# alibaba/VideoMV

Hardware: AMD Instinct MI355X
Metric: denoise-steps/sec, t2v 320x512x24 (latent 24x40x64), CFG 9.0, 50-step DDIM schedule (higher is better)
Workload: dtype fp16; 1 GPU; t2v_infer.yaml UNetSD_T2VBase 1.413B, 24 views, latent 40x64, 77 ctx tokens, 1 sample per GPU (cond+uncond batched); parallelism=replicas x1

## Files before the change

### include/vmv.h

```cpp
#ifndef VMV_H
#define VMV_H
#include <stdint.h>
#include <stddef.h>

#ifdef __cplusplus
extern "C" {
#endif

#define VMV_OK            0
#define VMV_EINVAL       -1
#define VMV_EALIGN       -2
#define VMV_ENULL        -3
#define VMV_ERANGE       -4
#define VMV_ECOMM        -5

#define VMV_ABI_VERSION   12
int vmv_abi_version(void);
#define VMV_ELEM_F16      0
#define VMV_ELEM_BF16     1
int vmv_elem_type(void);
int vmv_has_experiments(void);
int vmv_sizeof(int which);
const char* vmv_error_string(int code);

// ... 67 lines not shown
#define VMV_TILE_PP256x160 12
#define VMV_TILE_Q128x128 13
#define VMV_TILE_Q96x160  14
#define VMV_TILE_S256x128 15
#define VMV_TILE_S192x160 16
#define VMV_TILE_S256x160 17
#define VMV_TILE_A128x160 18
#define VMV_TILE_A128x128 19
#define VMV_TILE_X256x320 20
#define VMV_TILE_X256x256 21
#define VMV_TILE_X256x128 22
#define VMV_TILE_RS       23
#define VMV_TILE_RS512    24
#define VMV_TILE_RS256    25
#define VMV_TILE_HALO     26
#define VMV_TILE_TFR      27

#define VMV_TILE_TQA      28
#define VMV_TILE_W256x256 29

#define VMV_TILE_X512x128 30
#define VMV_TILE_Y256x128 31

#define VMV_TILE_TRS      32

int vmv_gemm(const VmvGemmParams* p, void* stream);
int vmv_gemm_tqa_ok(const VmvGemmParams* p);
int vmv_gemm_up4_ok(const VmvGemmParams* p);
int vmv_gemm_ln_inline_ok(const VmvGemmParams* p);
int vmv_gemm_rs_ok(const VmvGemmParams* p);
int vmv_gemm_tfr_ok(const VmvGemmParams* p);
int vmv_gemm_trs_ok(const VmvGemmParams* p);
int vmv_gemm_trs_blocks(const VmvGemmParams* p, int max_blocks, void* stream);
int vmv_gemm_pick_tile(const VmvGemmParams* p);
int vmv_gemm_validate(const VmvGemmParams* p);
int vmv_gemm_served_tile(const VmvGemmParams* p);
int vmv_gemm_tile_map(int bid, int tiles_m, int tiles_n, int gm, int* tile_m, int* tile_n);
int vmv_gemm_group_m(int tiles_m, int tiles_n, int BM, int BN, int conc);

typedef struct {
    int32_t M, C;
    const void* x; int32_t ldx;
    int32_t _pad0;
    const void* w1;
    const float* b1;
    const void* w2;
    const float* b2;
    const void* residual; int32_t ldr;
    float ln_eps;
    void* out; int32_t ldo;
    int32_t _pad1;
} VmvFfParams;
int vmv_ff_fused(const VmvFfParams* p, void* stream);
int vmv_ff_fused_ok(const VmvFfParams* p);

typedef struct {
    const void* x;
    const void* x1;
    int32_t ld, ld1;
    int32_t C0, C1;
    int32_t rows, rows_per_stat;
    int32_t chunk_rows;
    float* partial;
    const float* gamma;
    const float* beta;
    float eps;
    int32_t silu;
    void* y;
    int32_t ldy;
    int32_t fold_ranks;
    int64_t* totals;
    int64_t* totals_clear;
    int32_t clear_count;
    int32_t _pad;
} VmvGroupNormParams;

#define VMV_GN_REC 8
#define VMV_GN_NREP 8
int vmv_groupnorm_stats(const VmvGroupNormParams* p, void* stream);
int vmv_groupnorm_table(const VmvGroupNormParams* p, void* stream);
int vmv_groupnorm_apply(const VmvGroupNormParams* p, void* stream);
#define VMV_GN_FUSED_BYTES 131072
int vmv_groupnorm_fused(const VmvGroupNormParams* p, int32_t cols, void* stream);

typedef struct {
    const void* x; int32_t ldx;
    void* y; int32_t ldy;
    const float* gamma; const float* beta;
    int32_t rows, C;
    float eps;
    int32_t _pad;
    float* stats_out;
} VmvLayerNormParams;
int vmv_layernorm(const VmvLayerNormParams* p, void* stream);

typedef struct {
    const float* s; int32_t lds;
    void* p; int32_t ldp;
    int32_t rows, n;
    float scale;
    int32_t _pad;
} VmvSoftmaxParams;
int vmv_softmax_rows(const VmvSoftmaxParams* p, void* stream);

typedef struct {
    int64_t s_outer, s_inner, s_row;
    int32_t inner; int32_t _pad;
} VmvSeqMap;

typedef struct {
    const void* q; const void* k; const void* v; void* o;
    VmvSeqMap qm, km, vm, om;
    int32_t n_outer;
    int32_t kv_div;
    int32_t heads;
    int32_t Nq, Nk;
    float scale;
    int32_t head_dim;
    int32_t causal;
} VmvAttnParams;
int vmv_attention(const VmvAttnParams* p, void* stream);
#define VMV_ATTN_SHORT    1
#define VMV_ATTN_WAVE     2
#define VMV_ATTN_Q128     3
#define VMV_ATTN_Q256     4
#define VMV_ATTN_CAUSAL   5
#define VMV_ATTN_D32      6
#define VMV_ATTN_D128     7
int vmv_attention_served_kernel(const VmvAttnParams* p);

int vmv_latent_to_rows(const float* x, void* rows, int nb_src, int C, int F, int H, int W, int Cpad, int nrep,
                       void* stream);
int vmv_latent_to_rows_keep(const float* x, void* rows, int nb, int C, int F, int H, int W, int ld, int nrep, void* stream);
int vmv_rows_to_nchw(const void* rows, int rows_fp32, int ld, float* out, int n, int C, int HW, void* stream);

typedef struct {
    const float* eps_rows;
    int32_t ld;
    int32_t C, F, HW;
    float guide_scale;
    float c_recip, c_recipm1;
    float c_sqrt_ac, c_sqrt_1mac;
    float a_prev;
    int32_t v_pred;
    float* xt;
    float* x0_out;
    float clamp;
    float sigma;
    const float* noise;
} VmvDdimParams;
int vmv_cfg_ddim_step(const VmvDdimParams* p, void* stream);

int vmv_posterior_sample(const float* moments_rows, int ld, const float* noise, float* z, int n, int zc, int HW, float scale,
                         void* stream);
int vmv_emb_combine_silu(const float* temb, const float* cam, void* out, int rows, int C, int rows_per_t,
                         int cam_rows, void* stream);
int vmv_sinusoidal(const float* t, void* out_elem, int n, int dim, void* stream);

int vmv_i2v_temporal_adapter(const void* in, int ld_in, void* out, int ld_out, const float* w, int F, int HW, int nrep,
                             float scale, void* stream);
int vmv_adaptive_avgpool_rows(const void* in, int ld, void* out, int ldo, int n, int C, int IH, int IW, int OH, int OW,
                              void* stream);

int vmv_lgm_x0_views(const float* eps_rows, int ld, int branch, const float* xt, int C, int F, int HW, const int32_t* idx4,
                     float c_recip, float c_recipm1, float inv_scale, float* out, void* stream);
int vmv_lgm_pack_input(const float* decoded, const float* rays, float* out, int nviews, int HW, void* stream);
// ... 211 lines not shown
```

### videomv_amd/_lib.py

```python
import ctypes as C
import os

_HERE = os.path.dirname(os.path.abspath(__file__))
_ELEM_NAMES = {"fp16": "f16", "f16": "f16", "float16": "f16", "half": "f16", "bf16": "bf16", "bfloat16": "bf16"}
_elem = _ELEM_NAMES[os.environ.get("VMV_DTYPE", "fp16").lower()]
ELEM_F16, ELEM_BF16 = 0, 1


def set_elem(name: str):
    global _elem
    new = _ELEM_NAMES[str(name).lower()]
    if _lib is not None and new != _elem:
        raise RuntimeError(f"the {_elem} kernels are already loaded; set VMV_DTYPE / call set_elem() before first use")
    _elem = new


def elem_name() -> str:
    return "fp16" if _elem == "f16" else "bf16"


def elem():
    import torch
    return torch.float16 if _elem == "f16" else torch.bfloat16


def lib_path() -> str:
    return os.path.join(os.environ.get("VMV_LIB_DIR") or os.path.join(_HERE, "lib"), f"libvmv_hip_{_elem}.so")

VMV_MAX_SEGS = 24
SEG_LINEAR, SEG_SPATIAL, SEG_TEMPORAL = 0, 1, 2
EPI_NONE, EPI_GEGLU, EPI_TATTN = 0, 1, 2
ACT_NONE, ACT_SILU, ACT_GELU = 0, 1, 2
TILE_AUTO, TILE_128x128, TILE_128x160, TILE_128x64, TILE_64x64, TILE_256x128, TILE_256x160 = 0, 1, 2, 3, 4, 5, 6
TILE_G128x128, TILE_G128x160, TILE_P256x128, TILE_P256x160, TILE_PP256x128, TILE_PP256x160 = 7, 8, 9, 10, 11, 12
TILE_Q128x128, TILE_Q96x160 = 13, 14
TILE_S256x128, TILE_S192x160, TILE_S256x160 = 15, 16, 17
TILE_A128x160, TILE_A128x128 = 18, 19
TILE_X256x320, TILE_X256x256, TILE_X256x128 = 20, 21, 22
TILE_RS, TILE_RS512, TILE_RS256, TILE_HALO, TILE_TFR, TILE_TQA, TILE_W256x256, TILE_X512x128, TILE_Y256x128 = 23, 24, 25, 26, 27, 28, 29, 30, 31
TRS_TILE = 32
OP_GEMM, OP_GN_STATS, OP_GN_APPLY, OP_LAYERNORM, OP_ATTENTION, OP_SOFTMAX, OP_COPY, OP_GN_FUSED, OP_FF, OP_GN_TABLE, OP_COMM = 1, 2, 3, 4, 5, 6, 7, 8, 9, 10, 11
COMM_ALL_TO_ALL, COMM_ALL_GATHER, COMM_ID_BYTES = 0, 1, 128
ABI_VERSION = 12
ATTN_SHORT, ATTN_WAVE, ATTN_Q128, ATTN_Q256, ATTN_CAUSAL, ATTN_D32, ATTN_D128 = 1, 2, 3, 4, 5, 6, 7
GN_FUSED_BYTES = 131072


class GemmSeg(C.Structure):
    _fields_ = [("src", C.c_void_p), ("ld", C.c_int32), ("k", C.c_int32), ("mode", C.c_int32),
                ("d0", C.c_int32), ("d1", C.c_int32), ("_pad", C.c_int32)]


class GemmParams(C.Structure):
    _fields_ = [("M", C.c_int32), ("N", C.c_int32), ("nseg", C.c_int32), ("ktot", C.c_int32),
                ("seg", GemmSeg * VMV_MAX_SEGS),
                ("W", C.c_void_p), ("bias", C.c_void_p), ("rowvec", C.c_void_p),
                ("rowvec_div", C.c_int32), ("rowvec_ld", C.c_int32),
                ("residual", C.c_void_p), ("ldr", C.c_int32),
                ("epilogue", C.c_int32), ("act", C.c_int32), ("out_fp32", C.c_int32),
                ("out", C.c_void_p), ("ldo", C.c_int32),
                ("OH", C.c_int32), ("OW", C.c_int32), ("IH", C.c_int32), ("IW", C.c_int32),
                ("stride", C.c_int32), ("ups", C.c_int32),
                ("F", C.c_int32), ("P", C.c_int32),
                ("ksplit", C.c_int32), ("workspace", C.c_void_p),
                ("tile", C.c_int32), ("res_scale", C.c_float), ("rowstat", C.c_void_p), ("colsum", C.c_void_p),
                ("ln_eps", C.c_float), ("wgroup_rows", C.c_int32), ("wgroup_stride", C.c_int64),
                ("gn_table", C.c_void_p), ("gn_rows_per_stat", C.c_int32), ("gn_silu", C.c_int32), ("epi_scale", C.c_float),
                ("phased", C.c_int32)]


class GroupNormParams(C.Structure):
    _fields_ = [("x", C.c_void_p), ("x1", C.c_void_p), ("ld", C.c_int32), ("ld1", C.c_int32),
                ("C0", C.c_int32), ("C1", C.c_int32), ("rows", C.c_int32), ("rows_per_stat", C.c_int32),
                ("chunk_rows", C.c_int32), ("partial", C.c_void_p), ("gamma", C.c_void_p), ("beta", C.c_void_p),
                ("eps", C.c_float), ("silu", C.c_int32), ("y", C.c_void_p), ("ldy", C.c_int32), ("fold_ranks", C.c_int32),
                ("totals", C.c_void_p), ("totals_clear", C.c_void_p), ("clear_count", C.c_int32), ("_pad", C.c_int32)]


class FfParams(C.Structure):
    _fields_ = [("M", C.c_int32), ("C", C.c_int32), ("x", C.c_void_p), ("ldx", C.c_int32), ("_pad0", C.c_int32),
                ("w1", C.c_void_p), ("b1", C.c_void_p), ("w2", C.c_void_p), ("b2", C.c_void_p),
                ("residual", C.c_void_p), ("ldr", C.c_int32), ("ln_eps", C.c_float),
                ("out", C.c_void_p), ("ldo", C.c_int32), ("_pad1", C.c_int32)]


class GsParams(C.Structure):
    _fields_ = [("gaussians", C.c_void_p), ("N", C.c_int32), ("size", C.c_int32), ("view", C.c_void_p),
                ("view_proj", C.c_void_p), ("tan_half_fov", C.c_float), ("bg", C.c_float * 3),
                ("depth", C.c_void_p), ("xy", C.c_void_p), ("conic_opacity", C.c_void_p), ("rect", C.c_void_p),
                ("tiles_touched", C.c_void_p), ("offsets", C.c_void_p), ("scan_temp", C.c_void_p),
                ("scan_temp_bytes", C.c_size_t), ("keys", C.c_void_p), ("keys_sorted", C.c_void_p), ("vals", C.c_void_p),
                ("vals_sorted", C.c_void_p), ("num_rendered", C.c_int32), ("_pad", C.c_int32), ("sort_temp", C.c_void_p),
                ("sort_temp_bytes", C.c_size_t), ("ranges", C.c_void_p), ("out_color", C.c_void_p), ("out_alpha", C.c_void_p)]


class GsBatchParams(C.Structure):
    _fields_ = [("gaussians", C.c_void_p), ("B", C.c_int32), ("N", C.c_int32), ("V", C.c_int32), ("size", C.c_int32),
                ("views", C.c_void_p), ("view_projs", C.c_void_p), ("tan_half_fov", C.c_float), ("bg", C.c_float * 3),
                ("depth", C.c_void_p), ("xy", C.c_void_p), ("conic_opacity", C.c_void_p), ("rect", C.c_void_p),
                ("tiles_touched", C.c_void_p), ("offsets", C.c_void_p), ("scan_temp", C.c_void_p),
                ("scan_temp_bytes", C.c_size_t), ("keys", C.c_void_p), ("keys_sorted", C.c_void_p), ("vals", C.c_void_p),
                ("vals_sorted", C.c_void_p), ("num_rendered", C.c_int32), ("_pad", C.c_int32), ("sort_temp", C.c_void_p),
                ("sort_temp_bytes", C.c_size_t), ("ranges", C.c_void_p), ("out_color", C.c_void_p), ("out_alpha", C.c_void_p)]


class GsBackwardParams(C.Structure):
    _fields_ = [("pass_", GsBatchParams), ("final_T", C.c_void_p), ("n_contrib", C.c_void_p), ("dL_dimage", C.c_void_p),
                ("grad2d", C.c_void_p), ("grad_view", C.c_void_p), ("grad", C.c_void_p)]


class GsDepthParams(C.Structure):
    _fields_ = [("pass_", GsBatchParams), ("out_depth", C.c_void_p), ("out_median_depth", C.c_void_p)]


class GsAdamParams(C.Structure):
    _fields_ = [("params", C.c_void_p), ("m", C.c_void_p), ("v", C.c_void_p), ("grad", C.c_void_p), ("gaussians", C.c_void_p),
                ("n", C.c_int32), ("step", C.c_int32), ("lr", C.c_float * 5), ("beta1", C.c_float), ("beta2", C.c_float),
                ("eps", C.c_float)]


class GsSsimLossParams(C.Structure):
    _fields_ = [("image", C.c_void_p), ("target", C.c_void_p), ("planes", C.c_int32), ("height", C.c_int32), ("width", C.c_int32),
                ("lambda_dssim", C.c_float), ("dL_dimage", C.c_void_p), ("loss", C.c_void_p), ("workspace", C.c_void_p),
                ("workspace_bytes", C.c_size_t)]


class GsTsdfParams(C.Structure):
    _fields_ = [("depth", C.c_void_p), ("colour", C.c_void_p), ("views", C.c_void_p), ("n_views", C.c_int), ("size", C.c_int),
# ... 4 lines not shown
class GsMeshComponentsParams(C.Structure):
    _fields_ = [("faces", C.c_void_p), ("face_stride", C.c_int64), ("n_faces", C.c_int64), ("n_vertices", C.c_int64),
                ("label", C.c_void_p), ("face_count", C.c_void_p), ("status", C.c_void_p)]


class GsMeshBakeParams(C.Structure):
    _fields_ = [("verts", C.c_void_p), ("vert_colours", C.c_void_p), ("faces", C.c_void_p), ("face_stride", C.c_int64),
                ("n_faces", C.c_int64), ("n_vertices", C.c_int64), ("depth", C.c_void_p), ("colour", C.c_void_p), ("views", C.c_void_p),
                ("n_views", C.c_int32), ("size", C.c_int32), ("tan_half_fov", C.c_float), ("z_min", C.c_float), ("depth_tol", C.c_float),
                ("cos_min", C.c_float), ("patch", C.c_int32), ("tex_size", C.c_int32), ("out", C.c_void_p), ("plane_stride", C.c_int64),
                ("status", C.c_void_p)]


MESH_STATUS_RANGE, MESH_STATUS_GAVE_UP = 1, 2


class CopyParams(C.Structure):
    _fields_ = [("src", C.c_void_p), ("dst", C.c_void_p), ("n0", C.c_int32), ("n1", C.c_int32), ("n2", C.c_int32),
                ("inner16", C.c_int32), ("ss0", C.c_int64), ("ss1", C.c_int64), ("ss2", C.c_int64)]


class CommParams(C.Structure):
    _fields_ = [("comm", C.c_void_p), ("kind", C.c_int32), ("_pad", C.c_int32), ("send", C.c_void_p), ("recv", C.c_void_p),
                ("bytes", C.c_int64)]


class LayerNormParams(C.Structure):
    _fields_ = [("x", C.c_void_p), ("ldx", C.c_int32), ("y", C.c_void_p), ("ldy", C.c_int32),
                ("gamma", C.c_void_p), ("beta", C.c_void_p), ("rows", C.c_int32), ("C", C.c_int32),
                ("eps", C.c_float), ("_pad", C.c_int32), ("stats_out", C.c_void_p)]


class SeqMap(C.Structure):
    _fields_ = [("s_outer", C.c_int64), ("s_inner", C.c_int64), ("s_row", C.c_int64),
                ("inner", C.c_int32), ("_pad", C.c_int32)]


class AttnParams(C.Structure):
    _fields_ = [("q", C.c_void_p), ("k", C.c_void_p), ("v", C.c_void_p), ("o", C.c_void_p),
                ("qm", SeqMap), ("km", SeqMap), ("vm", SeqMap), ("om", SeqMap),
                ("n_outer", C.c_int32), ("kv_div", C.c_int32), ("heads", C.c_int32),
                ("Nq", C.c_int32), ("Nk", C.c_int32), ("scale", C.c_float), ("head_dim", C.c_int32), ("causal", C.c_int32)]


class SoftmaxParams(C.Structure):
    _fields_ = [("s", C.c_void_p), ("lds", C.c_int32), ("p", C.c_void_p), ("ldp", C.c_int32),
                ("rows", C.c_int32), ("n", C.c_int32), ("scale", C.c_float), ("_pad", C.c_int32)]


class DdimParams(C.Structure):
    _fields_ = [("eps_rows", C.c_void_p), ("ld", C.c_int32), ("C", C.c_int32), ("F", C.c_int32), ("HW", C.c_int32),
                ("guide_scale", C.c_float), ("c_recip", C.c_float), ("c_recipm1", C.c_float),
                ("c_sqrt_ac", C.c_float), ("c_sqrt_1mac", C.c_float), ("a_prev", C.c_float),
                ("v_pred", C.c_int32), ("xt", C.c_void_p), ("x0_out", C.c_void_p),
                ("clamp", C.c_float), ("sigma", C.c_float), ("noise", C.c_void_p)]


_P = C.c_void_p
SYMBOLS = {
    "vmv_abi_version": (C.c_int, []),
    "vmv_elem_type": (C.c_int, []),
    "vmv_sizeof": (C.c_int, [C.c_int]),
    "vmv_error_string": (C.c_char_p, [C.c_int]),
    "vmv_gemm": (C.c_int, [C.POINTER(GemmParams), _P]),
    "vmv_gemm_ln_inline_ok": (C.c_int, [C.POINTER(GemmParams)]),
    "vmv_gemm_rs_ok": (C.c_int, [C.POINTER(GemmParams)]),
    "vmv_gemm_tfr_ok": (C.c_int, [C.POINTER(GemmParams)]),
    "vmv_gemm_tqa_ok": (C.c_int, [C.POINTER(GemmParams)]),
    "vmv_gemm_trs_ok": (C.c_int, [C.POINTER(GemmParams)]),
    "vmv_gemm_trs_blocks": (C.c_int, [C.POINTER(GemmParams), C.c_int, _P]),
    "vmv_gemm_up4_ok": (C.c_int, [C.POINTER(GemmParams)]),
    "vmv_has_experiments": (C.c_int, []),
    "vmv_ff_fused": (C.c_int, [C.POINTER(FfParams), _P]),
    "vmv_ff_fused_ok": (C.c_int, [C.POINTER(FfParams)]),
    "vmv_gemm_pick_tile": (C.c_int, [C.POINTER(GemmParams)]),
    "vmv_gemm_validate": (C.c_int, [C.POINTER(GemmParams)]),
    "vmv_gemm_served_tile": (C.c_int, [C.POINTER(GemmParams)]),
    "vmv_gemm_tile_map": (C.c_int, [C.c_int, C.c_int, C.c_int, C.c_int, C.POINTER(C.c_int), C.POINTER(C.c_int)]),
    "vmv_gemm_group_m": (C.c_int, [C.c_int, C.c_int, C.c_int, C.c_int, C.c_int]),
    "vmv_groupnorm_stats": (C.c_int, [C.POINTER(GroupNormParams), _P]),
    "vmv_groupnorm_apply": (C.c_int, [C.POINTER(GroupNormParams), _P]),
    "vmv_groupnorm_table": (C.c_int, [C.POINTER(GroupNormParams), _P]),
    "vmv_groupnorm_fused": (C.c_int, [C.POINTER(GroupNormParams), C.c_int32, _P]),
    "vmv_layernorm": (C.c_int, [C.POINTER(LayerNormParams), _P]),
    "vmv_attention": (C.c_int, [C.POINTER(AttnParams), _P]),
    "vmv_attention_served_kernel": (C.c_int, [C.POINTER(AttnParams)]),
    "vmv_softmax_rows": (C.c_int, [C.POINTER(SoftmaxParams), _P]),
    "vmv_permute_copy": (C.c_int, [C.POINTER(CopyParams), _P]),
    "vmv_gaussian_activation": (C.c_int, [_P, C.c_int, _P, C.c_int, _P, _P]),
    "vmv_lgm_x0_views": (C.c_int, [_P, C.c_int, C.c_int, _P, C.c_int, C.c_int, C.c_int, _P, C.c_float, C.c_float, C.c_float, _P, _P]),
    "vmv_lgm_pack_input": (C.c_int, [_P, _P, _P, C.c_int, C.c_int, _P]),
    "vmv_lgm_render_to_vae": (C.c_int, [_P, _P, C.c_int, C.c_int, C.c_int, _P]),
    "vmv_ddim_x0_step": (C.c_int, [_P, _P, _P, C.c_long, C.c_float, C.c_float, C.c_float, C.c_float, C.c_float, C.c_float, _P, _P]),
    "vmv_gs_workspace_bytes": (C.c_int, [C.c_int, C.c_int, C.POINTER(C.c_size_t), C.POINTER(C.c_size_t)]),
    "vmv_gs_preprocess": (C.c_int, [C.POINTER(GsParams), _P]),
    "vmv_gs_render": (C.c_int, [C.POINTER(GsParams), _P]),
    "vmv_gs_batch_key_bits": (C.c_int, [C.c_int, C.c_int]),
    "vmv_gs_batch_workspace_bytes": (C.c_int, [C.c_int, C.c_int, C.c_int, C.POINTER(C.c_size_t), C.POINTER(C.c_size_t)]),
    "vmv_gs_batch_preprocess": (C.c_int, [C.POINTER(GsBatchParams), _P]),
    "vmv_gs_batch_render": (C.c_int, [C.POINTER(GsBatchParams), _P]),
    "vmv_gs_batch_render_depth": (C.c_int, [C.POINTER(GsDepthParams), _P]),
    "vmv_gs_batch_render_state": (C.c_int, [C.POINTER(GsBackwardParams), _P]),
    "vmv_gs_batch_backward": (C.c_int, [C.POINTER(GsBackwardParams), _P]),
    "vmv_gs_image_loss": (C.c_int, [_P, _P, C.c_long, _P, _P, _P, _P]),
    "vmv_gs_adam_step": (C.c_int, [C.POINTER(GsAdamParams), _P]),
    "vmv_gs_ssim_loss_workspace_bytes": (C.c_int, [C.c_int, C.c_int, C.c_int, C.POINTER(C.c_size_t)]),
    "vmv_gs_ssim_loss": (C.c_int, [C.POINTER(GsSsimLossParams), _P]),
    "vmv_gs_tsdf_integrate": (C.c_int, [C.POINTER(GsTsdfParams), _P]),
    "vmv_gs_mesh_components": (C.c_int, [C.POINTER(GsMeshComponentsParams), _P]),
    "vmv_gs_mesh_bake": (C.c_int, [C.POINTER(GsMeshBakeParams), _P]),
    "vmv_latent_to_rows": (C.c_int, [_P, _P, C.c_int, C.c_int, C.c_int, C.c_int, C.c_int, C.c_int, C.c_int, _P]),
    "vmv_latent_to_rows_keep": (C.c_int, [_P, _P, C.c_int, C.c_int, C.c_int, C.c_int, C.c_int, C.c_int, C.c_int, _P]),
    "vmv_i2v_temporal_adapter": (C.c_int, [_P, C.c_int, _P, C.c_int, _P, C.c_int, C.c_int, C.c_int, C.c_float, _P]),
    "vmv_adaptive_avgpool_rows": (C.c_int, [_P, C.c_int, _P, C.c_int, C.c_int, C.c_int, C.c_int, C.c_int, C.c_int, C.c_int, _P]),
    "vmv_rows_to_nchw": (C.c_int, [_P, C.c_int, C.c_int, _P, C.c_int, C.c_int, C.c_int, _P]),
    "vmv_cfg_ddim_step": (C.c_int, [C.POINTER(DdimParams), _P]),
    "vmv_posterior_sample": (C.c_int, [_P, C.c_int, _P, _P, C.c_int, C.c_int, C.c_int, C.c_float, _P]),
    "vmv_emb_combine_silu": (C.c_int, [_P, _P, _P, C.c_int, C.c_int, C.c_int, C.c_int, _P]),
    "vmv_sinusoidal": (C.c_int, [_P, _P, C.c_int, C.c_int, _P]),
    "vmv_plan_create": (_P, []),
    "vmv_plan_destroy": (None, [_P]),
    "vmv_plan_add": (C.c_int, [_P, C.c_int, _P, C.c_size_t]),
    "vmv_plan_size": (C.c_int, [_P]),
    "vmv_plan_run": (C.c_int, [_P, _P]),
    "vmv_plan_run_range": (C.c_int, [_P, C.c_int, C.c_int, _P]),
    "vmv_plan_capture": (_P, [_P, _P]),
    "vmv_graph_launch": (C.c_int, [_P, _P]),
    "vmv_graph_nodes": (C.c_int, [_P]),
    "vmv_graph_destroy": (None, [_P]),
    "vmv_comm_load": (C.c_int, [C.c_char_p]),
    "vmv_comm_loaded": (C.c_int, []),
    "vmv_comm_unique_id": (C.c_int, [_P]),
    "vmv_comm_create": (_P, [_P, C.c_int, C.c_int]),
    "vmv_comm_create_sim": (_P, [C.c_int, C.c_int]),
    "vmv_comm_destroy": (None, [_P]),
    "vmv_comm_world": (C.c_int, [_P]),
    "vmv_comm_rank": (C.c_int, [_P]),
    "vmv_comm_is_sim": (C.c_int, [_P]),
    "vmv_comm_run": (C.c_int, [C.POINTER(CommParams), _P]),
}

_lib = None


def load():
    global _lib
    if _lib is not None:
        return _lib
    LIB_PATH = lib_path()
    if not os.path.exists(LIB_PATH):
        raise RuntimeError(
            f"{LIB_PATH} is missing: build the HIP extension first (python -c 'import __graft_entry__ as g; "
            f"g.build()' or make -C videomv_amd/csrc).  There is no CPU fallback for the hot path.")
    lib = C.CDLL(LIB_PATH)
    for name, (res, args) in SYMBOLS.items():
        fn = getattr(lib, name)
        fn.restype = res
        fn.argtypes = args
    if lib.vmv_abi_version() != ABI_VERSION:
        raise RuntimeError(f"{LIB_PATH}: ABI version mismatch")
    if lib.vmv_elem_type() != (ELEM_F16 if _elem == "f16" else ELEM_BF16):
        raise RuntimeError(f"{LIB_PATH} was built for another element type")
    for which, st in ((OP_GEMM, GemmParams), (OP_GN_STATS, GroupNormParams), (OP_LAYERNORM, LayerNormParams),
                      (OP_ATTENTION, AttnParams), (OP_SOFTMAX, SoftmaxParams), (OP_COPY, CopyParams), (OP_FF, FfParams), (OP_COMM, CommParams), (103, GsParams), (104, GsBatchParams), (105, GsBackwardParams), (106, GsAdamParams), (107, GsSsimLossParams), (108, GsDepthParams), (109, GsTsdfParams), (110, GsMeshComponentsParams), (111, GsMeshBakeParams), (100, DdimParams), (101, GemmSeg), (102, SeqMap)):
        if lib.vmv_sizeof(which) != C.sizeof(st):
            raise RuntimeError(f"struct layout drift for {st.__name__}: C {lib.vmv_sizeof(which)} vs ctypes "
# ... 14 lines not shown
```

### videomv_amd/csrc/norm.hip

```cpp
#include "common.h"
#include <type_traits>

namespace {

constexpr float GN_LO = 1099511627776.0f;

VMV_DEV void gn_add2(unsigned long long* rec, int which, float v) {
    const float fl = floorf(v);
    atomicAdd(rec + which, (unsigned long long)(long long)fl);
    atomicAdd(rec + 2 + which, (unsigned long long)(long long)((v - fl) * GN_LO));
}

struct GnSlots {
    int TPR, RPP;
    __host__ __device__ explicit GnSlots(int slots) : TPR(slots < 256 ? slots : 256), RPP(256 / TPR) {}
};
struct GnLane : GnSlots {
    int rl, cl;
    bool active;
    __device__ explicit GnLane(int slots) : GnSlots(slots), rl((int)threadIdx.x / TPR), cl((int)threadIdx.x - rl * TPR), active(rl < RPP) {}
};
struct GnSrc { const uint16_t* base; long ld; };
VMV_DEV GnSrc gn_src(const VmvGroupNormParams& p, int c) {
    const bool first = c < p.C0;
    return {first ? reinterpret_cast<const uint16_t*>(p.x) + c : reinterpret_cast<const uint16_t*>(p.x1) + (c - p.C0),
            first ? p.ld : p.ld1};
}
VMV_DEV float gn_pilot(const VmvGroupNormParams& p, long row, int c) {
    const GnSrc s = gn_src(p, c);
    return elem_to_f32(s.base[row * s.ld]);
}
template <int U, typename F>
VMV_DEV void gn_walk(const uint16_t* base, long ld, long& r, long row_end, int RPP, F f) {
    for (; r + (long)(U - 1) * RPP < row_end; r += (long)U * RPP) {
        u32x4_t v[U];
#pragma unroll
        for (int k = 0; k < U; ++k) v[k] = *reinterpret_cast<const u32x4_t*>(base + (r + (long)k * RPP) * ld);
#pragma unroll
        for (int k = 0; k < U; ++k) f(v[k], r + (long)k * RPP);
    }
}
VMV_DEV void gn_scale_shift(float* scale, float* shift, const float* s_mean, const float* s_rstd, const VmvGroupNormParams& p,
                            int c0, int n, int cpg) {
    for (int c = threadIdx.x; c < n; c += 256) {
        const int g = c / cpg;
        const float sc = s_rstd[g] * p.gamma[c0 + c];
        scale[c] = sc;
        shift[c] = p.beta[c0 + c] - s_mean[g] * sc;
    }
}
struct GnAffine {
    float a[8], b[8];
    VMV_DEV GnAffine(const float* scale, const float* shift) {
#pragma unroll
        for (int e = 0; e < 8; ++e) { a[e] = scale[e]; b[e] = shift[e]; }
    }
    template <bool SILU>
    VMV_DEV u32x4_t apply(const u32x4_t& v) const {
        float f[8];
        unpack8(v, f);
#pragma unroll
        for (int e = 0; e < 8; ++e) {
            f[e] = f[e] * a[e] + b[e];
            if constexpr (SILU) f[e] = silu_f(f[e]);
        }
        return pack8(f);
    }
};

__global__ __launch_bounds__(256) void gn_stats_kernel(const VmvGroupNormParams p, const int nchunk) {
    VMV_KERNEL_ENTER();
    extern __shared__ __attribute__((aligned(16))) float sh[];
    const int C = p.C0 + p.C1;
    const int CS = C >> 3;
    const GnLane L(CS);
    const int RPP = L.RPP, rl = L.rl;
    const int tid = threadIdx.x;
    const int stat = blockIdx.y, chunk = blockIdx.x;
    const long row0 = (long)stat * p.rows_per_stat + (long)chunk * p.chunk_rows;
    long row_end = row0 + p.chunk_rows;
    const long stat_end = (long)(stat + 1) * p.rows_per_stat;
    if (row_end > stat_end) row_end = stat_end;
    float* lsum = sh;
// ... 167 lines not shown
        for (int e = 0; e < 8; ++e) s[e] = 0.f;
        if (active) {
            const GnSrc src = gn_src(p, c0 + cs * 8);
            const uint16_t* base = src.base;
            const long ld = src.ld;
            int r = rl;
            for (; r + (GNF_UNR - 1) * RPP < rows; r += GNF_UNR * RPP) {
                u32x4_t v[GNF_UNR];
#pragma unroll
                for (int k = 0; k < GNF_UNR; ++k) v[k] = *reinterpret_cast<const u32x4_t*>(base + (row0 + r + k * RPP) * ld);
#pragma unroll
                for (int k = 0; k < GNF_UNR; ++k) {
                    stage[(size_t)(r + k * RPP) * SW + cs] = v[k];
                    float f[8];
                    unpack8(v[k], f);
#pragma unroll
                    for (int e = 0; e < 8; ++e) s[e] += f[e];
                }
            }
            for (; r < rows; r += RPP) {
                const u32x4_t v = *reinterpret_cast<const u32x4_t*>(base + (row0 + r) * ld);
                stage[(size_t)r * SW + cs] = v;
                float f[8];
                unpack8(v, f);
#pragma unroll
                for (int e = 0; e < 8; ++e) s[e] += f[e];
            }
#pragma unroll
            for (int e = 0; e < 8; ++e) red[rl * CW + cs * 8 + e] = s[e];
        }
    }
    __syncthreads();
    const float n = (float)rows * (float)cpg;
    auto group_totals = [&](float* dst, auto finish) {
        float cs = 0.f;
        if (tid < CW)
            for (int r = 0; r < RPP; ++r) cs += red[r * CW + tid];
        __syncthreads();
        if (tid < CW) red[tid] = cs;
        __syncthreads();
        const int wv = tid >> 6, ln = tid & 63;
        for (int g = wv; g < G; g += 4) {
            float s = 0.f;
            for (int c = ln; c < cpg; c += 64) s += red[g * cpg + c];
            s = wave_sum(s);
            if (ln == 0) dst[g] = finish(s);
        }
        __syncthreads();
    };
    group_totals(s_mean, [&](float s) { return s / n; });
    for (int cs = cl; cs < SW; cs += TPR) {
        if (active) {
            float mu[8], q[8];
#pragma unroll
            for (int e = 0; e < 8; ++e) { mu[e] = s_mean[(cs * 8 + e) / cpg]; q[e] = 0.f; }
            for (int r = rl; r < rows; r += RPP) {
                float f[8];
                unpack8(stage[(size_t)r * SW + cs], f);
#pragma unroll
                for (int e = 0; e < 8; ++e) { const float d = f[e] - mu[e]; q[e] += d * d; }
            }
#pragma unroll
            for (int e = 0; e < 8; ++e) red[rl * CW + cs * 8 + e] = q[e];
        }
    }
    __syncthreads();
    group_totals(s_rstd, [&](float q) { return rsqrtf(q / n + p.eps); });
    gn_scale_shift(scale, shift, s_mean, s_rstd, p, c0, CW, cpg);
    __syncthreads();
    uint16_t* y = reinterpret_cast<uint16_t*>(p.y);
    if (active) {
        for (int cs = cl; cs < SW; cs += TPR) {
            const GnAffine af(scale + cs * 8, shift + cs * 8);
            uint16_t* dst = y + c0 + cs * 8;
            auto run = [&](auto silu_tag) {
                for (int r = rl; r < rows; r += RPP)
                    *reinterpret_cast<u32x4_t*>(dst + (row0 + r) * p.ldy) = af.apply<decltype(silu_tag)::value>(stage[(size_t)r * SW + cs]);
            };
            if (p.silu) run(std::true_type{}); else run(std::false_type{});
        }
    }
}

constexpr int LN_MAX_IT = 5;
template <int LPR>
__global__ __launch_bounds__(256) void layernorm_kernel(const VmvLayerNormParams p) {
    VMV_KERNEL_ENTER();
    constexpr int RPW = 64 / LPR;
    const int lane = threadIdx.x & 63;
    const int sub = lane % LPR;
    const long row = ((long)blockIdx.x * 4 + (threadIdx.x >> 6)) * RPW + lane / LPR;
    const bool live = row < p.rows;
    const int CS = p.C >> 3;
    const uint16_t* x = reinterpret_cast<const uint16_t*>(p.x) + (live ? row : 0) * p.ldx;
    float f[LN_MAX_IT][8];
    float s = 0.f;
#pragma unroll
    for (int it = 0; it < LN_MAX_IT; ++it) {
        const int cs = sub + it * LPR;
        if (cs < CS) {
            unpack8(*reinterpret_cast<const u32x4_t*>(x + cs * 8), f[it]);
#pragma unroll
            for (int e = 0; e < 8; ++e) s += f[it][e];
        }
    }
#pragma unroll
    for (int o = LPR / 2; o > 0; o >>= 1) s += __shfl_xor(s, o, 64);
    const float mean = s / (float)p.C;
    float q = 0.f;
#pragma unroll
    for (int it = 0; it < LN_MAX_IT; ++it) {
        const int cs = sub + it * LPR;
        if (cs < CS) {
#pragma unroll
            for (int e = 0; e < 8; ++e) { const float d = f[it][e] - mean; q += d * d; }
        }
    }
#pragma unroll
    for (int o = LPR / 2; o > 0; o >>= 1) q += __shfl_xor(q, o, 64);
    const float rstd = rsqrtf(q / (float)p.C + p.eps);
    if (!live) return;
    if (p.stats_out) {
        if (sub == 0) *reinterpret_cast<float2*>(p.stats_out + row * 2) = make_float2(mean, rstd);
        return;
    }
    uint16_t* y = reinterpret_cast<uint16_t*>(p.y) + row * p.ldy;
#pragma unroll
    for (int it = 0; it < LN_MAX_IT; ++it) {
        const int cs = sub + it * LPR;
        if (cs < CS) {
            const int c = cs * 8;
            const f32x4_t g0 = *reinterpret_cast<const f32x4_t*>(p.gamma + c);
            const f32x4_t g1 = *reinterpret_cast<const f32x4_t*>(p.gamma + c + 4);
            const f32x4_t b0 = *reinterpret_cast<const f32x4_t*>(p.beta + c);
            const f32x4_t b1 = *reinterpret_cast<const f32x4_t*>(p.beta + c + 4);
            float o[8];
            o[0] = (f[it][0] - mean) * rstd * g0.x + b0.x; o[1] = (f[it][1] - mean) * rstd * g0.y + b0.y;
            o[2] = (f[it][2] - mean) * rstd * g0.z + b0.z; o[3] = (f[it][3] - mean) * rstd * g0.w + b0.w;
            o[4] = (f[it][4] - mean) * rstd * g1.x + b1.x; o[5] = (f[it][5] - mean) * rstd * g1.y + b1.y;
            o[6] = (f[it][6] - mean) * rstd * g1.z + b1.z; o[7] = (f[it][7] - mean) * rstd * g1.w + b1.w;
            *reinterpret_cast<u32x4_t*>(y + c) = pack8(o);
        }
    }
}

__global__ __launch_bounds__(256) void softmax_rows_kernel(const VmvSoftmaxParams p) {
    VMV_KERNEL_ENTER();
    const int lane = threadIdx.x & 63;
    const long row = (long)blockIdx.x * 4 + (threadIdx.x >> 6);
    if (row >= p.rows) return;
    const float* s = p.s + row * p.lds;
    const float sc = p.scale * 1.44269504088896341f;
    const int n4 = p.n >> 2;
    float mx = -3.0e38f;
    for (int i = lane; i < n4; i += 64) {
        const f32x4_t v = *reinterpret_cast<const f32x4_t*>(s + 4 * i);
        mx = fmaxf(fmaxf(fmaxf(mx, v.x), fmaxf(v.y, v.z)), v.w);
    }
#pragma unroll
    for (int o = 32; o > 0; o >>= 1) mx = fmaxf(mx, __shfl_xor(mx, o, 64));
    const float m2 = mx * sc;
    float sum = 0.f;
    for (int i = lane; i < n4; i += 64) {
        const f32x4_t v = *reinterpret_cast<const f32x4_t*>(s + 4 * i);
        sum += __builtin_amdgcn_exp2f(v.x * sc - m2) + __builtin_amdgcn_exp2f(v.y * sc - m2) +
               __builtin_amdgcn_exp2f(v.z * sc - m2) + __builtin_amdgcn_exp2f(v.w * sc - m2);
    }
    const float inv = 1.0f / wave_sum(sum);
    uint16_t* out = reinterpret_cast<uint16_t*>(p.p) + row * p.ldp;
    for (int i = lane; i < n4; i += 64) {
        const f32x4_t v = *reinterpret_cast<const f32x4_t*>(s + 4 * i);
        u32x2_t w;
        w.x = pack_elem2(__builtin_amdgcn_exp2f(v.x * sc - m2) * inv, __builtin_amdgcn_exp2f(v.y * sc - m2) * inv);
        w.y = pack_elem2(__builtin_amdgcn_exp2f(v.z * sc - m2) * inv, __builtin_amdgcn_exp2f(v.w * sc - m2) * inv);
        *reinterpret_cast<u32x2_t*>(out + 4 * i) = w;
    }
}

int gn_check(const VmvGroupNormParams& p, bool ws) {
    if (!p.x || (ws && !p.partial && !p.totals)) return VMV_ENULL;
    const int C = p.C0 + p.C1;
    if (C <= 0 || (C & 31) || (p.C0 & 7) || (p.C1 & 7)) return VMV_EINVAL;
    if (p.C1 > 0 && !p.x1) return VMV_ENULL;
    if (p.rows <= 0 || p.rows_per_stat <= 0 || (p.rows % p.rows_per_stat) || (ws && p.chunk_rows <= 0)) return VMV_EINVAL;
    if (!vmv_aligned16(p.x) || (p.ld & 7) || (p.C1 > 0 && (!vmv_aligned16(p.x1) || (p.ld1 & 7)))) return VMV_EALIGN;
    if (C > 4096) return VMV_ERANGE;
    return VMV_OK;
}
int gn_check_out(const VmvGroupNormParams& p, bool table) {
    if (!p.y || !p.gamma || !p.beta) return VMV_ENULL;
    if (table && p.silu) return VMV_EINVAL;
    if (!vmv_aligned16(p.y) || (!table && (p.ldy & 7)) || !vmv_aligned16(p.gamma) || !vmv_aligned16(p.beta)) return VMV_EALIGN;
    return VMV_OK;
}
struct GnGrid { int nstat, nchunk; };
GnGrid gn_grid(const VmvGroupNormParams& p) { return {p.rows / p.rows_per_stat, (p.rows_per_stat + p.chunk_rows - 1) / p.chunk_rows}; }

int gn_apply_launch(const VmvGroupNormParams* pp, void* stream, bool table) {
    if (!pp) return VMV_ENULL;
    const VmvGroupNormParams& p = *pp;
    if (const int rc = gn_check(p, true)) return rc;
    if (const int rc = gn_check_out(p, table)) return rc;
    if (p.fold_ranks > 1 && !p.totals) return VMV_EINVAL;
    const int C = p.C0 + p.C1;
    const GnGrid g = gn_grid(p);
    int apply_rows = (65536 / (C * 2));
    if (apply_rows < 1 || table) apply_rows = 1;
    const int nblk = table ? 1 : (p.rows_per_stat + apply_rows - 1) / apply_rows;
    hipLaunchKernelGGL(gn_apply_kernel, dim3(nblk, g.nstat), dim3(256), (size_t)(2 * C + 64) * sizeof(float),
                       reinterpret_cast<hipStream_t>(stream), p, g.nchunk, apply_rows, g.nstat, table ? reinterpret_cast<float*>(p.y) : nullptr);
    return vmv_launch_status();
}

}

extern "C" int vmv_groupnorm_stats(const VmvGroupNormParams* pp, void* stream) {
    if (!pp) return VMV_ENULL;
    const VmvGroupNormParams& p = *pp;
    if (const int rc = gn_check(p, true)) return rc;
    const int C = p.C0 + p.C1;
    const GnGrid g = gn_grid(p);
    const size_t shbytes = ((size_t)2 * GnSlots(C >> 3).RPP * C + 32) * sizeof(float);
    if (p.totals && (((uintptr_t)p.totals) & 7)) return VMV_EALIGN;
    hipLaunchKernelGGL(gn_stats_kernel, dim3(g.nchunk, g.nstat), dim3(256), shbytes, reinterpret_cast<hipStream_t>(stream), p, g.nchunk);
    return vmv_launch_status();
}

extern "C" int vmv_groupnorm_apply(const VmvGroupNormParams* pp, void* stream) { return gn_apply_launch(pp, stream, false); }
extern "C" int vmv_groupnorm_table(const VmvGroupNormParams* pp, void* stream) { return gn_apply_launch(pp, stream, true); }

extern "C" int vmv_groupnorm_fused(const VmvGroupNormParams* pp, int32_t cols, void* stream) {
    if (!pp) return VMV_ENULL;
    const VmvGroupNormParams& p = *pp;
    if (const int rc = gn_check(p, false)) return rc;
    if (const int rc = gn_check_out(p, false)) return rc;
    const int C = p.C0 + p.C1, cpg = C >> 5;
    if (cols <= 0 || (cols & 7) || (cols % cpg) || (C % cols)) return VMV_EINVAL;
    if (cols > 256) return VMV_ERANGE;
    if (p.fold_ranks > 1) return VMV_EINVAL;
    if ((long)p.rows_per_stat * cols * 2 > VMV_GN_FUSED_BYTES) return VMV_ERANGE;
    const size_t shbytes = (size_t)p.rows_per_stat * cols * 2 + (size_t)(GnSlots(cols >> 3).RPP * cols + 2 * cols + 64) * sizeof(float);
    if (shbytes > 160 * 1024) return VMV_ERANGE;
    static std::atomic<unsigned long long> attr{0};
    if (const int rc_attr = vmv_lds_attr_once(attr, reinterpret_cast<const void*>(&gn_fused_kernel), 160 * 1024)) return rc_attr;
    hipLaunchKernelGGL(gn_fused_kernel, dim3(C / cols, p.rows / p.rows_per_stat), dim3(256), shbytes,
                       reinterpret_cast<hipStream_t>(stream), p, cols);
    return vmv_launch_status();
}

extern "C" int vmv_layernorm(const VmvLayerNormParams* pp, void* stream) {
    if (!pp) return VMV_ENULL;
    const VmvLayerNormParams& p = *pp;
    if (!p.x) return VMV_ENULL;
    if (!p.stats_out && (!p.y || !p.gamma || !p.beta)) return VMV_ENULL;
    if (p.rows <= 0 || p.C <= 0 || (p.C & 7)) return VMV_EINVAL;
    if (p.C > LN_MAX_IT * 64 * 8) return VMV_ERANGE;
    if (!vmv_aligned16(p.x) || (p.ldx & 7)) return VMV_EALIGN;
    if (p.stats_out) { if (((uintptr_t)p.stats_out) & 7) return VMV_EALIGN; }
    else if (!vmv_aligned16(p.y) || (p.ldy & 7) || !vmv_aligned16(p.gamma) || !vmv_aligned16(p.beta)) return VMV_EALIGN;
    const int CS = p.C >> 3;
    hipStream_t st = reinterpret_cast<hipStream_t>(stream);
    auto go = [&](auto lpr_tag) {
        constexpr int LPR = decltype(lpr_tag)::value;
        const int rows_per_block = 4 * (64 / LPR);
        const int blocks = (p.rows + rows_per_block - 1) / rows_per_block;
        hipLaunchKernelGGL(layernorm_kernel<LPR>, dim3(blocks), dim3(256), 0, st, p);
    };
    if (CS <= 8 * LN_MAX_IT) go(std::integral_constant<int, 8>{});
    else if (CS <= 16 * LN_MAX_IT) go(std::integral_constant<int, 16>{});
    else if (CS <= 32 * LN_MAX_IT) go(std::integral_constant<int, 32>{});
    else go(std::integral_constant<int, 64>{});
    return vmv_launch_status();
}

extern "C" int vmv_softmax_rows(const VmvSoftmaxParams* pp, void* stream) {
    if (!pp) return VMV_ENULL;
    const VmvSoftmaxParams& p = *pp;
    if (!p.s || !p.p) return VMV_ENULL;
    if (p.rows <= 0 || p.n <= 0 || (p.n & 3) || p.scale <= 0.f) return VMV_EINVAL;
    if (!vmv_aligned16(p.s) || (p.lds & 3) || (((uintptr_t)p.p) & 7) || (p.ldp & 3)) return VMV_EALIGN;
    hipLaunchKernelGGL(softmax_rows_kernel, dim3((p.rows + 3) / 4), dim3(256), 0, reinterpret_cast<hipStream_t>(stream), p);
    return vmv_launch_status();
}
```

Before: 21.26 denoise-steps/s.

## Add register-resident fused GroupNorm kernel with XCD-aware slab split

```diff
diff --git a/include/vmv.h b/include/vmv.h
--- a/include/vmv.h
+++ b/include/vmv.h
@@ -173,6 +173,11 @@
 int vmv_groupnorm_apply(const VmvGroupNormParams* p, void* stream);
 #define VMV_GN_FUSED_BYTES 131072
 int vmv_groupnorm_fused(const VmvGroupNormParams* p, int32_t cols, void* stream);
+#define VMV_GNF_STAGED 0
+#define VMV_GNF_FORM(d) ((d) & 0xff)
+#define VMV_GNF_SPLIT(d) ((d) >> 8)
+int vmv_groupnorm_fused_served(const VmvGroupNormParams* p, int32_t cols, int32_t ncu);
+int vmv_groupnorm_fused_form(const VmvGroupNormParams* p, int32_t cols, int32_t form, int32_t split, void* stream);
 
 typedef struct {
     const void* x; int32_t ldx;
diff --git a/videomv_amd/_lib.py b/videomv_amd/_lib.py
--- a/videomv_amd/_lib.py
+++ b/videomv_amd/_lib.py
@@ -44,6 +44,7 @@
 ABI_VERSION = 12
 ATTN_SHORT, ATTN_WAVE, ATTN_Q128, ATTN_Q256, ATTN_CAUSAL, ATTN_D32, ATTN_D128 = 1, 2, 3, 4, 5, 6, 7
 GN_FUSED_BYTES = 131072
+GNF_STAGED, GNF_BUCKETS = 0, (4, 8, 12, 20, 26, 32)
 
 
 class GemmSeg(C.Structure):
@@ -214,6 +215,8 @@
     "vmv_groupnorm_apply": (C.c_int, [C.POINTER(GroupNormParams), _P]),
     "vmv_groupnorm_table": (C.c_int, [C.POINTER(GroupNormParams), _P]),
     "vmv_groupnorm_fused": (C.c_int, [C.POINTER(GroupNormParams), C.c_int32, _P]),
+    "vmv_groupnorm_fused_served": (C.c_int, [C.POINTER(GroupNormParams), C.c_int32, C.c_int32]),
+    "vmv_groupnorm_fused_form": (C.c_int, [C.POINTER(GroupNormParams), C.c_int32, C.c_int32, C.c_int32, _P]),
     "vmv_layernorm": (C.c_int, [C.POINTER(LayerNormParams), _P]),
     "vmv_attention": (C.c_int, [C.POINTER(AttnParams), _P]),
     "vmv_attention_served_kernel": (C.c_int, [C.POINTER(AttnParams)]),
diff --git a/videomv_amd/csrc/norm.hip b/videomv_amd/csrc/norm.hip
--- a/videomv_amd/csrc/norm.hip
+++ b/videomv_amd/csrc/norm.hip
@@ -1,4 +1,5 @@
 #include "common.h"
+#include "gemm_rs_common.h"
 #include <type_traits>
 
 namespace {
@@ -332,6 +333,121 @@
     }
 }
 
+constexpr int GNR_BOUNDS[] = {4, 8, 12, 20, 26, 32};
+template <typename F>
+VMV_DEV void gnr_group_totals(const float* red, float* col, float* dst, const int CW, const int RPP, const int G, const int cpg, F finish) {
+    const int tid = threadIdx.x;
+    if (tid < CW) {
+        float cs = 0.f;
+        for (int r = 0; r < RPP; ++r) cs += red[r * CW + tid];
+        col[tid] = cs;
+    }
+    __syncthreads();
+    const int wv = tid >> 6, ln = tid & 63;
+    for (int g = wv; g < G; g += 4) {
+        float s = 0.f;
+        for (int c = ln; c < cpg; c += 64) s += col[g * cpg + c];
+        s = wave_sum(s);
+        if (ln == 0) dst[g] = finish(s);
+    }
+    __syncthreads();
+}
+
+template <int NR>
+__global__ __launch_bounds__(256) void gn_fused_reg_kernel(const VmvGroupNormParams p, const int CW, const int split, const int nslab) {
+    VMV_KERNEL_ENTER();
+    extern __shared__ __attribute__((aligned(16))) float sh[];
+    const int xcd = blockIdx.x & 7, idx = blockIdx.x >> 3;
+    const int sb = (idx / split) * 8 + xcd, part = idx % split;
+    if (sb >= nslab) return;
+    const int slab = vmvg::xcd_logical(sb, nslab);
+    const int C = p.C0 + p.C1;
+    const int cpg = C >> 5;
+    const int G = CW / cpg;
+    const int ncx = C / CW;
+    const int stat = slab / ncx, c0 = (slab - stat * ncx) * CW;
+    const GnLane L(CW >> 3);
+    const int RPP = L.RPP, rl = L.rl, cs = L.cl;
+    const bool active = L.active;
+    const int rows = p.rows_per_stat;
+    const long row0 = (long)stat * rows;
+    float* red = sh;
+    float* col = red + RPP * CW;
+    float* scale = col + CW;
+    float* shift = scale + CW;
+    float* s_mean = shift + CW;
+    float* s_rstd = s_mean + 32;
+    float gam = 0.f, bet = 0.f;
+    if ((int)threadIdx.x < CW) { gam = p.gamma[c0 + threadIdx.x]; bet = p.beta[c0 + threadIdx.x]; }
+    u32x4_t v[NR];
+    if (active) {
+        const GnSrc src = gn_src(p, c0 + cs * 8);
+        const bool has = rl < rows;
+        const int klast = has ? (rows - 1 - rl) / RPP : 0;
+        const uint16_t* base = src.base + (row0 + (has ? rl : 0)) * src.ld;
+        const long step = (long)RPP * src.ld;
+#pragma unroll
+        for (int k = 0; k < NR; ++k) v[k] = *reinterpret_cast<const u32x4_t*>(base + (long)(k < klast ? k : klast) * step);
+        float s[8];
+#pragma unroll
+        for (int e = 0; e < 8; ++e) s[e] = 0.f;
+#pragma unroll
+        for (int k = 0; k < NR; ++k) {
+            if (rl + k * RPP < rows) {
+                float f[8];
+                unpack8(v[k], f);
+#pragma unroll
+                for (int e = 0; e < 8; ++e) s[e] += f[e];
+            }
+        }
+#pragma unroll
+        for (int e = 0; e < 8; ++e) red[rl * CW + cs * 8 + e] = s[e];
+    }
+    __syncthreads();
+    const float n = (float)rows * (float)cpg;
+    gnr_group_totals(red, col, s_mean, CW, RPP, G, cpg, [&](float s) { return s / n; });
+    if (active) {
+        float mu[8], q[8];
+#pragma unroll
+        for (int e = 0; e < 8; ++e) { mu[e] = s_mean[(cs * 8 + e) / cpg]; q[e] = 0.f; }
+#pragma unroll
+        for (int k = 0; k < NR; ++k) {
+            if (rl + k * RPP < rows) {
+                float f[8];
+                unpack8(v[k], f);
+#pragma unroll
+                for (int e = 0; e < 8; ++e) { const float d = f[e] - mu[e]; q[e] = __builtin_fmaf(d, d, q[e]); }
+            }
+        }
+#pragma unroll
+        for (int e = 0; e < 8; ++e) red[rl * CW + cs * 8 + e] = q[e];
+    }
+    __syncthreads();
+    gnr_group_totals(red, col, s_rstd, CW, RPP, G, cpg, [&](float q) { return rsqrtf(q / n + p.eps); });
+    if ((int)threadIdx.x < CW) {
+        const int g = threadIdx.x / cpg;
+        const float sc = s_rstd[g] * gam;
+        scale[threadIdx.x] = sc;
+        shift[threadIdx.x] = bet - s_mean[g] * sc;
+    }
+    __syncthreads();
+    if (active) {
+        const int per = (rows + split - 1) / split;
+        const int lo = part * per, hi = lo + per < rows ? lo + per : rows;
+        const GnAffine af(scale + cs * 8, shift + cs * 8);
+        uint16_t* dst = reinterpret_cast<uint16_t*>(p.y) + c0 + cs * 8 + (row0 + rl) * p.ldy;
+        const long stepy = (long)RPP * p.ldy;
+        auto run = [&](auto silu_tag) {
+#pragma unroll
+            for (int k = 0; k < NR; ++k) {
+                const int r = rl + k * RPP;
+                if (r >= lo && r < hi) *reinterpret_cast<u32x4_t*>(dst + k * stepy) = af.apply<decltype(silu_tag)::value>(v[k]);
+            }
+        };
+        if (p.silu) run(std::true_type{}); else run(std::false_type{});
+    }
+}
+
 constexpr int LN_MAX_IT = 5;
 template <int LPR>
 __global__ __launch_bounds__(256) void layernorm_kernel(const VmvLayerNormParams p) {
@@ -479,7 +595,9 @@
 extern "C" int vmv_groupnorm_apply(const VmvGroupNormParams* pp, void* stream) { return gn_apply_launch(pp, stream, false); }
 extern "C" int vmv_groupnorm_table(const VmvGroupNormParams* pp, void* stream) { return gn_apply_launch(pp, stream, true); }
 
-extern "C" int vmv_groupnorm_fused(const VmvGroupNormParams* pp, int32_t cols, void* stream) {
+namespace {
+
+int gnf_decide(const VmvGroupNormParams* pp, int cols, int ncu, int force_form, int force_split) {
     if (!pp) return VMV_ENULL;
     const VmvGroupNormParams& p = *pp;
     if (const int rc = gn_check(p, false)) return rc;
@@ -489,13 +607,74 @@
     if (cols > 256) return VMV_ERANGE;
     if (p.fold_ranks > 1) return VMV_EINVAL;
     if ((long)p.rows_per_stat * cols * 2 > VMV_GN_FUSED_BYTES) return VMV_ERANGE;
-    const size_t shbytes = (size_t)p.rows_per_stat * cols * 2 + (size_t)(GnSlots(cols >> 3).RPP * cols + 2 * cols + 64) * sizeof(float);
+    const int RPP = GnSlots(cols >> 3).RPP;
+    const size_t shbytes = (size_t)p.rows_per_stat * cols * 2 + (size_t)(RPP * cols + 2 * cols + 64) * sizeof(float);
     if (shbytes > 160 * 1024) return VMV_ERANGE;
-    static std::atomic<unsigned long long> attr{0};
-    if (const int rc_attr = vmv_lds_attr_once(attr, reinterpret_cast<const void*>(&gn_fused_kernel), 160 * 1024)) return rc_attr;
-    hipLaunchKernelGGL(gn_fused_kernel, dim3(C / cols, p.rows / p.rows_per_stat), dim3(256), shbytes,
-                       reinterpret_cast<hipStream_t>(stream), p, cols);
+    if (force_split != 0 && force_split != 1 && force_split != 2 && force_split != 4 && force_split != 8) return VMV_EINVAL;
+    const int nr = (p.rows_per_stat + RPP - 1) / RPP;
+    int bucket = 0;
+    for (const int b : GNR_BOUNDS)
+        if (nr <= b) { bucket = b; break; }
+    if (force_form > 0 && !bucket) return VMV_EINVAL;
+    const bool pays = nr > 2;
+    if (force_form == VMV_GNF_STAGED || !bucket || (force_form < 0 && !pays)) {
+        if (force_split > 1) return VMV_EINVAL;
+        return VMV_GNF_STAGED | (1 << 8);
+    }
+    int split = force_split;
+    if (!split) {
+        if (ncu <= 0) ncu = vmvg::rs_ncu_whole_xcds();
+        const long nslab = (long)(C / cols) * (p.rows / p.rows_per_stat);
+        split = 1;
+        while (split < 4 && nslab * split * 2 <= ncu && (p.rows_per_stat + 2 * split - 1) / (2 * split) >= RPP) split *= 2;
+    }
+    return bucket | (split << 8);
+}
+
+template <int NR>
+void gnf_launch_reg(const VmvGroupNormParams& p, int cols, int split, hipStream_t st) {
+    const int nslab = (p.C0 + p.C1) / cols * (p.rows / p.rows_per_stat);
+    const size_t shbytes = (size_t)(GnSlots(cols >> 3).RPP * cols + 3 * cols + 64) * sizeof(float);
+    hipLaunchKernelGGL(gn_fused_reg_kernel<NR>, dim3(split * 8 * ((nslab + 7) / 8)), dim3(256), shbytes, st, p, cols, split, nslab);
+}
+
+int gnf_launch(const VmvGroupNormParams* pp, int cols, int decision, void* stream) {
+    if (decision < 0) return decision;
+    const VmvGroupNormParams& p = *pp;
+    hipStream_t st = reinterpret_cast<hipStream_t>(stream);
+    const int form = VMV_GNF_FORM(decision), split = VMV_GNF_SPLIT(decision);
+    switch (form) {
+        case VMV_GNF_STAGED: {
+            const size_t shbytes = (size_t)p.rows_per_stat * cols * 2 + (size_t)(GnSlots(cols >> 3).RPP * cols + 2 * cols + 64) * sizeof(float);
+            static std::atomic<unsigned long long> attr{0};
+            if (const int rc_attr = vmv_lds_attr_once(attr, reinterpret_cast<const void*>(&gn_fused_kernel), 160 * 1024)) return rc_attr;
+            hipLaunchKernelGGL(gn_fused_kernel, dim3((p.C0 + p.C1) / cols, p.rows / p.rows_per_stat), dim3(256), shbytes, st, p, cols);
+            break;
+        }
+        case 4: gnf_launch_reg<4>(p, cols, split, st); break;
+        case 8: gnf_launch_reg<8>(p, cols, split, st); break;
+        case 12: gnf_launch_reg<12>(p, cols, split, st); break;
+        case 20: gnf_launch_reg<20>(p, cols, split, st); break;
+        case 26: gnf_launch_reg<26>(p, cols, split, st); break;
+        case 32: gnf_launch_reg<32>(p, cols, split, st); break;
+        default: return VMV_EINVAL;
+    }
     return vmv_launch_status();
+}
+
+}
+
+extern "C" int vmv_groupnorm_fused_served(const VmvGroupNormParams* pp, int32_t cols, int32_t ncu) {
+    return gnf_decide(pp, cols, ncu < 0 ? 0 : ncu, -1, 0);
+}
+
+extern "C" int vmv_groupnorm_fused_form(const VmvGroupNormParams* pp, int32_t cols, int32_t form, int32_t split, void* stream) {
+    if (form < 0 || split < 0) return VMV_EINVAL;
+    return gnf_launch(pp, cols, gnf_decide(pp, cols, 0, form, split), stream);
+}
+
+extern "C" int vmv_groupnorm_fused(const VmvGroupNormParams* pp, int32_t cols, void* stream) {
+    return gnf_launch(pp, cols, gnf_decide(pp, cols, 0, -1, 0), stream);
 }
 
 extern "C" int vmv_layernorm(const VmvLayerNormParams* pp, void* stream) {
```

New measurement: 21.37 denoise-steps/s, median of 6. Within noise of the previous version (+0.5%).
